# AE-HYU/monte_carlo_localization

Hardware: AMD Instinct MI355X
Metric: MCL updates/sec (particle*beam/s) (higher is better)
Workload: dtype f64; 1 GPU; 4194304 particles/GPU x 1081 beams, Spielberg_map (2000x2000 @ 0.05796), initial cloud N((0.0, 0.0, 0.0),(0.5 m,0.5 m,0.4 rad)) (tracking regime), action (0.05, 0.0, 0.01), stock sensor/motion params, multinomial resampling, Philox seed 42; the timed updates follow 5 warm-up updates (the particle set has resampled to motion-noise width); particles_total=4194304, beams=1081, parallelism=single GPU

## Files before the change

### monte_carlo_localization_amd/csrc/mcl_engine.hip

```cpp
#include "../../include/mcl_hip_engine.h"

#include <hip/hip_runtime.h>
#include <hip/hip_ext.h>
#include <rocprim/device/device_radix_sort.hpp>

#include <algorithm>
#include <chrono>
#include <cmath>
#include <cstdio>
#include <cstring>
#include <string>
#include <vector>

#include "mcl_engine_internal.h"
#include "mcl_kernels.h"
#include "mcl_host_math.h"
#include "mcl_lfield.h"

static_assert(MCL_WEDGES == mcl::kWedges || MCL_KWEDGES != 16, "include/mcl_hip_engine.h and csrc/mcl_wedge.h disagree");

using namespace mcl_host;

namespace {

thread_local std::string g_create_error;

int ensure_lt(mcl_engine *h)
{
    size_t need = (size_t)(h->P + 1) * h->bpad;
    if (need > h->lt_capacity) {
        dfree(h->d_Lt);
        HIPCHK(h, hipMalloc(&h->d_Lt, 2 * need * sizeof(float)));
        h->lt_capacity = need;
    }
    h->ltd_cols = (h->B + 2 * h->beam_margin + 64) & ~63;
    const size_t need_d = (size_t)mcl::sweep_table_rows(h->P) * h->ltd_cols;
    if (need_d > h->ltd_capacity) {
        dfree(h->d_Ltd);
        HIPCHK(h, hipMalloc(&h->d_Ltd, need_d * sizeof(double)));
        h->ltd_capacity = need_d;
        h->ltd_ready = false;
    }
    return MCL_OK;
}

void build_ltd(mcl_engine *h);

int weight_stats(mcl_engine *h, bool from_log, const double *d_max_override, bool defer_sums = false)
{
    const int64_t n = h->N;
    const double *src = from_log ? h->d_logw : h->d_w;
    const double *max_parts = nullptr;
    if (!d_max_override) {
        if (!(from_log && h->max_partials_ready))
            hipLaunchKernelGGL(mcl::k_reduce_max, dim3(mcl::kRedBlocks), dim3(mcl::kRedThreads), 0, h->stream, src, n, h->d_maxpart);
        max_parts = h->d_maxpart;
    }
    h->max_partials_ready = false;
    hipLaunchKernelGGL(mcl::k_weights, dim3(mcl::kRedBlocks), dim3(mcl::kRedThreads), 0, h->stream, src, from_log ? 1 : 0,
                       d_max_override ? d_max_override : h->d_scalars, h->d_x[h->cur], h->d_y[h->cur], h->d_th[h->cur], n, h->d_w, h->d_q, h->d_part,
                       (from_log && h->cfg.resample_neff_permille > 0) ? h->d_carry[h->carry_idx ^ 1] : (double *)nullptr,
                       max_parts, mcl::kRedBlocks);
    h->carry_pending = from_log && h->cfg.resample_neff_permille > 0;
    if (!from_log) h->carry_valid = false;
    if (defer_sums) h->sums_pending = true;
    else hipLaunchKernelGGL(mcl::k_final_sums, dim3(1), dim3(mcl::kRedThreads), 0, h->stream, h->d_part, mcl::kRedBlocks, h->d_scalars);
    HIPCHK(h, hipGetLastError());
    return MCL_OK;
}

int fetch_scalars(mcl_engine *h)
{
    HIPCHK(h, hipMemcpyAsync(h->h_result, h->d_result, kResultWords * 8, hipMemcpyDeviceToHost, h->stream));
    HIPCHK(h, hipStreamSynchronize(h->stream));
    unpack_result(h);
    return MCL_OK;
}

bool sweep_hybrid(const mcl_engine *h)
{
    return h->sweep_global && h->env_sweep_hybrid != 0 && h->rec_ok && h->sweep_hyb_layout_ok && h->d_beam_err != nullptr &&
           h->d_distw != nullptr && h->d_distg != nullptr && (size_t)mcl::kSwWinBytes + (size_t)h->ltd_cols * 8 <= 80 * 1024 - 64;
}

bool sweep_far_expected(const mcl_engine *h) { return h->far_fresh || h->h_result[15] >= mcl::kFarWindowedMin / 2; }
bool sweep_hybrid_decide(mcl_engine *h)
{
    if (!sweep_hybrid(h)) return false;
    if (h->env_sweep_hybrid == 2) return true;
    if (h->far_fresh) { h->hyb_backoff = 0; h->hyb_skip = 0; return false; }
    if (h->last_sweep_global == 2) {
        if (h->h_result[15] >= mcl::kFarWindowedMin / 2) { h->hyb_backoff = h->hyb_backoff ? std::min(32, 2 * h->hyb_backoff) : 1; h->hyb_skip = h->hyb_backoff; }
        else h->hyb_backoff = 0;
    }
    if (h->hyb_skip > 0) { --h->hyb_skip; return false; }
    return true;
}

int sweep_play(const mcl_engine *h, bool hybrid)
{
    if (hybrid) return mcl::kSwSide - (mcl::kSwHybReach + 2) - 3;
    if (h->sweep_global) return 1 << 20;
    return mcl::kSwSide - (h->P + 2) - 3;
}

int64_t max_sweep_units(int64_t n) { return (n + mcl::kSwUnit - 1) / mcl::kSwUnit + mcl::kSwMaxCuts + 2; }

int launch_sweep_plan(mcl_engine *h, int64_t n, int nwg, int g, bool hybrid)
{
    const int ngroups = mcl::kWedges / g;
    const size_t need = (size_t)max_sweep_units(n) * ngroups;
    if (need > h->items_capacity) {
        dfree(h->d_items); dfree(h->d_centres);
        h->items_capacity = 0;
        HIPCHK(h, hipMalloc(&h->d_items, need * sizeof(int4)));
// ... 284 lines not shown
            a.far_sorted = h->d_far_sorted;
            a.far_windowed = sweep_far_expected(h) ? 1 : 0;
            h->far_fresh = false;
            a.far_list = h->d_far_list; a.far_count = h->d_result + 15;
        }
        const bool sweep_hyb = sweep && sweep_hyb_now;
        const bool sweep_glob = sweep && h->sweep_global && !sweep_hyb;
        const bool sweep_rec = sweep && h->rec_ok && h->sweep_rec_layout_ok && h->d_beam_err != nullptr &&
                               (size_t)mcl::kSwWinBytes + (size_t)h->ltd_cols * 8 <= 80 * 1024 - 64;
        const bool sweep_pairs = sweep_rec && !sweep_hyb && (h->env_sweep_pairs >= 0 ? h->env_sweep_pairs != 0 : (sweep_glob || a.far_windowed != 0));
        size_t qlds = sweep ? (sweep_glob ? 0 : (size_t)mcl::kSwWinBytes) + (sweep_rec ? (size_t)h->ltd_cols * 8 : 0) : (size_t)h->qside * h->qside;
        h->last_sweep_global = sweep_glob ? 1 : (sweep_hyb ? 2 : 0); h->last_sweep_rec = sweep_rec ? 1 : 0; h->last_sweep_pairs = (sweep_rec && (sweep_glob || sweep_pairs)) ? 1 : 0;
        dim3 qg((unsigned)nseg);
        unsigned long long *d_dbg = nullptr;
        const char *dbgpath = h->env_debug_wg.empty() ? nullptr : h->env_debug_wg.c_str();
        if (dbgpath) { HIPCHK(h, hipMalloc(&d_dbg, (size_t)qg.x * 32)); HIPCHK(h, hipMemset(d_dbg, 0, (size_t)qg.x * 32)); a.dbg = d_dbg; }
        dim3 gfar((unsigned)std::max<int64_t>(1, std::min<int64_t>(4 * (int64_t)h->num_cu, (n + 15) / 16)));
        const int fix_split = std::max(1, std::min(16, (8 * h->num_cu) / std::max(nseg, 1)));
        if (!sweep) HIPCHK(h, hipEventRecord(h->ev[EV_K0], h->stream));
        if (count) {
            if (sweep_hyb) hipExtLaunchKernelGGL((mcl::k_rays_sweep<true, false, true, false, true>), qg, b, qlds, h->stream, nullptr, h->ev[EV_K1], 0, a);
            else if (sweep_glob && sweep_rec) hipExtLaunchKernelGGL((mcl::k_rays_sweep<true, true, true, true>), qg, b, qlds, h->stream, nullptr, h->ev[EV_K1], 0, a);
            else if (sweep_glob) hipExtLaunchKernelGGL((mcl::k_rays_sweep<true, true>), qg, b, qlds, h->stream, nullptr, h->ev[EV_K1], 0, a);
            else if (sweep && sweep_rec && sweep_pairs) hipExtLaunchKernelGGL((mcl::k_rays_sweep<true, false, true, true>), qg, b, qlds, h->stream, nullptr, h->ev[EV_K1], 0, a);
            else if (sweep && sweep_rec) hipExtLaunchKernelGGL((mcl::k_rays_sweep<true, false, true>), qg, b, qlds, h->stream, nullptr, h->ev[EV_K1], 0, a);
            else if (sweep) hipExtLaunchKernelGGL((mcl::k_rays_sweep<true>), qg, b, qlds, h->stream, nullptr, h->ev[EV_K1], 0, a);
#ifdef MCL_LEGACY_RAY_KERNELS
            else if (cell) hipLaunchKernelGGL((mcl::k_rays_cell<true>), qg, b, qlds, h->stream, a);
            else hipLaunchKernelGGL((mcl::k_rays_quad<true>), qg, b, qlds, h->stream, a);
#endif
            if (!sweep) HIPCHK(h, hipEventRecord(h->ev[EV_K1], h->stream));
            if (sweep && a.far_windowed) { const int rcw = launch_far_windowed(h, a, n, true); if (rcw) return rcw; }
            hipLaunchKernelGGL((mcl::k_rays_far<true>), gfar, b, 0, h->stream, a);
            hipLaunchKernelGGL((mcl::k_rays_fix<true>), dim3(nseg * fix_split), dim3(256), 0, h->stream, a);
            hipLaunchKernelGGL((mcl::k_rays_exact<true>), dim3(2 * h->num_cu), dim3(256), 0, h->stream, a);
        } else {
            if (sweep_hyb) hipExtLaunchKernelGGL((mcl::k_rays_sweep<false, false, true, false, true>), qg, b, qlds, h->stream, nullptr, h->ev[EV_K1], 0, a);
            else if (sweep_glob && sweep_rec) hipExtLaunchKernelGGL((mcl::k_rays_sweep<false, true, true, true>), qg, b, qlds, h->stream, nullptr, h->ev[EV_K1], 0, a);
            else if (sweep_glob) hipExtLaunchKernelGGL((mcl::k_rays_sweep<false, true>), qg, b, qlds, h->stream, nullptr, h->ev[EV_K1], 0, a);
            else if (sweep && sweep_rec && sweep_pairs) hipExtLaunchKernelGGL((mcl::k_rays_sweep<false, false, true, true>), qg, b, qlds, h->stream, nullptr, h->ev[EV_K1], 0, a);
            else if (sweep && sweep_rec) hipExtLaunchKernelGGL((mcl::k_rays_sweep<false, false, true>), qg, b, qlds, h->stream, nullptr, h->ev[EV_K1], 0, a);
            else if (sweep) hipExtLaunchKernelGGL((mcl::k_rays_sweep<false>), qg, b, qlds, h->stream, nullptr, h->ev[EV_K1], 0, a);
#ifdef MCL_LEGACY_RAY_KERNELS
            else if (cell) hipLaunchKernelGGL((mcl::k_rays_cell<false>), qg, b, qlds, h->stream, a);
            else hipLaunchKernelGGL((mcl::k_rays_quad<false>), qg, b, qlds, h->stream, a);
#endif
            if (!sweep) HIPCHK(h, hipEventRecord(h->ev[EV_K1], h->stream));
            if (sweep && a.far_windowed) { const int rcw = launch_far_windowed(h, a, n, false); if (rcw) return rcw; }
            hipLaunchKernelGGL((mcl::k_rays_far<false>), gfar, b, 0, h->stream, a);
            hipLaunchKernelGGL((mcl::k_rays_fix<false>), dim3(nseg * fix_split), dim3(256), 0, h->stream, a);
            hipLaunchKernelGGL((mcl::k_rays_exact<false>), dim3(2 * h->num_cu), dim3(256), 0, h->stream, a);
        }
        if (sweep) {
            hipExtLaunchKernelGGL(mcl::k_combine_logw, dim3(mcl::kRedBlocks), dim3(256), 0, h->stream, nullptr, h->ev[EV_RAYS], 0, n, h->d_perm, h->d_logw_acc,
                                  h->d_logw, h->d_maxpart, h->d_fix_count, nseg, segcap, h->d_fix_over);
            h->ev_rays_bound = true;
            h->max_partials_ready = true;
        } else {
            hipLaunchKernelGGL(mcl::k_fix_overflow, dim3(1), dim3(256), 0, h->stream, h->d_fix_count, nseg, segcap, h->d_fix_over);
            hipLaunchKernelGGL(mcl::k_gather_logw, dim3((unsigned)((n + 255) / 256)), dim3(256), 0, h->stream, h->d_logw_acc, n, h->d_logw);
        }
        if (d_dbg) {
            std::vector<unsigned long long> hd((size_t)qg.x * 4);
            HIPCHK(h, hipStreamSynchronize(h->stream));
            HIPCHK(h, hipMemcpy(hd.data(), d_dbg, hd.size() * 8, hipMemcpyDeviceToHost));
            if (FILE *f = fopen(dbgpath, "wb")) { fwrite(hd.data(), 8, hd.size(), f); fclose(f); }
            (void)hipFree(d_dbg);
        }
        h->last_quad = true;
    } else if (count) {
        hipLaunchKernelGGL((mcl::k_rays_skip<1, true>), g, b, lds, h->stream, a);
    } else {
        switch (R) {
        case 1: hipLaunchKernelGGL((mcl::k_rays_skip<1, false>), g, b, lds, h->stream, a); break;
        case 2: hipLaunchKernelGGL((mcl::k_rays_skip<2, false>), g, b, lds, h->stream, a); break;
        case 3: hipLaunchKernelGGL((mcl::k_rays_skip<3, false>), g, b, lds, h->stream, a); break;
        default: hipLaunchKernelGGL((mcl::k_rays_skip<4, false>), g, b, lds, h->stream, a); break;
        }
    }
    if (!windows && !h->capturing && !direct_table) HIPCHK(h, hipEventRecord(h->ev[EV_K1], h->stream));
    h->last_mode = mode;
    h->prep_folded = false;
    h->layout_stale_used = false; h->keys_done = false;
    if (!h->capturing) h->pc_ready = false;
    HIPCHK(h, hipGetLastError());
    return MCL_OK;
}

void stage_observation(mcl_engine *h, const float *obs, int stride)
{
    h->ltd_ready = false;
    for (int j = 0; j < h->B; ++j) h->h_obs[j] = obs[(size_t)j * stride];
}

void build_ltd(mcl_engine *h)
{
    dim3 gd((h->ltd_cols + 255) / 256, mcl::sweep_table_rows(h->P));
    hipLaunchKernelGGL(mcl::k_build_ltd, gd, dim3(256), 0, h->stream, h->d_L, h->d_obs_idx, h->B, h->ltd_cols, h->P, h->beam_margin, h->d_Ltd);
    h->ltd_ready = true;
}

int upload_observation(mcl_engine *h)
{
    HIPCHK(h, hipMemcpyAsync(h->d_obs, h->h_obs, (size_t)h->B * sizeof(float), hipMemcpyHostToDevice, h->stream));
    int rc = h->capturing ? MCL_OK : ensure_lt(h);
    if (rc) return rc;
    dim3 g((h->bpad + 255) / 256, h->P + 1);
    hipLaunchKernelGGL(mcl::k_obs_build_lt, g, dim3(256), 0, h->stream, h->d_obs, h->res, h->P, h->d_L, h->B, h->bpad, h->d_obs_idx, h->d_Lt,
// ... 143 lines not shown
    const int nb = mcl_host::lf_used_beams(h, obs, stride, h->h_lf_beams);
    if (nb > 0)
        HIPCHK(h, hipMemcpyAsync(h->d_lf_beams, h->h_lf_beams, (size_t)nb * sizeof(double2), hipMemcpyHostToDevice, h->stream));
    HIPCHK(h, hipEventRecord(h->ev[EV_QUERY], h->stream));
    HIPCHK(h, hipEventRecord(h->ev[EV_K0], h->stream));
    const int rc = mcl_host::launch_lfield_on(h, h->d_x[h->cur], h->d_y[h->cur], h->d_th[h->cur], n, h->d_lf_beams, nb, h->d_logw);
    if (rc != MCL_OK) return rc;
    HIPCHK(h, hipEventRecord(h->ev[EV_K1], h->stream));
    h->max_partials_ready = false;
    h->last_quad = false;
    h->last_lf = true;
    return MCL_OK;
}

}

int mcl_host::fail(mcl_engine *h, int code, const char *msg) { if (h) h->err = msg; return code; }
int mcl_host::fail(mcl_engine *h, int code, const std::string &msg) { return fail(h, code, msg.c_str()); }

std::string &mcl_host::create_error() { return g_create_error; }

bool mcl_host::ready(mcl_engine *h, bool need_particles)
{
    return h && h->have_map && h->B > 0 && (!need_particles || h->have_particles);
}

float mcl_host::elapsed(hipEvent_t a, hipEvent_t b)
{
    float ms = 0.f;
    (void)hipEventElapsedTime(&ms, a, b);
    return ms;
}

void mcl_host::graph_reset(mcl_engine *h)
{
    for (int k = 0; k < 2; ++k)
        if (h->graph_exec[k]) { (void)hipGraphExecDestroy(h->graph_exec[k]); h->graph_exec[k] = nullptr; }
    h->graph_warm = false;
    h->prep_cache_valid = false; h->prep_folded = false;
    h->layout_valid = false; h->layout_stale_used = false; h->keys_done = false;
    h->pc_ready = false;
}

int mcl_host::scan_weights(mcl_engine *h, const uint64_t *d_q, uint64_t *d_cdf, int64_t n, uint64_t offset, uint64_t *d_total)
{
    int nb = (int)((n + mcl::kScanTile - 1) / mcl::kScanTile);
    mcl::CompactOut co{};
    const bool own = d_q == h->d_q && d_cdf == h->d_cdf && offset == 0 && !h->env_no_compact && h->d_ccdf;
    if (own) {
        co.block_cnt = h->d_blockcnt; co.ccdf = h->d_ccdf; co.cidx = h->d_cidx; co.crec = h->d_crec; co.ctop = h->d_ctop;
        co.x = h->d_x[h->cur]; co.y = h->d_y[h->cur]; co.th = h->d_th[h->cur];
        co.cap = (uint32_t)h->compact_cap; co.total = h->d_result + 16;
    }
    hipLaunchKernelGGL(mcl::k_scan_partials, dim3(nb), dim3(mcl::kScanThreads), 0, h->stream, d_q, n, h->d_blocktot, co.block_cnt);
    const bool fold = h->sums_pending && d_q == h->d_q;
    hipLaunchKernelGGL(mcl::k_scan_spine, dim3(1), dim3(1024), 0, h->stream, h->d_blocktot, nb, offset, d_total, co.block_cnt, co.total,
                       fold ? h->d_part : (const double *)nullptr, mcl::kRedBlocks, h->d_scalars);
    if (fold) h->sums_pending = false;
    const size_t nlead = (size_t)((n + 15) >> mcl::kLeaderShift) + 1;
    if (nlead > h->leaders_capacity) {
        graph_reset(h);
        dfree(h->d_leaders);
        HIPCHK(h, hipMalloc(&h->d_leaders, nlead * 8));
        h->leaders_capacity = nlead;
    }
    if (h->bind_sensor_event && own && !h->capturing) {
        hipExtLaunchKernelGGL(mcl::k_scan_final, dim3(nb), dim3(mcl::kScanThreads), 0, h->stream, nullptr, h->ev[EV_SENSOR], 0, d_q, n, h->d_blocktot, d_cdf,
                              h->d_leaders, co);
        h->ev_sensor_bound = true; h->bind_sensor_event = false;
    } else {
        hipLaunchKernelGGL(mcl::k_scan_final, dim3(nb), dim3(mcl::kScanThreads), 0, h->stream, d_q, n, h->d_blocktot, d_cdf, h->d_leaders, co);
    }
    HIPCHK(h, hipGetLastError());
    h->blocktot_for = d_cdf; h->blocktot_n = n;
    if (d_cdf == h->d_cdf) { h->compact_n = -1; h->compact_pending = own; h->list_epoch++; }
    return MCL_OK;
}

void mcl_host::unpack_result(mcl_engine *h)
{
    std::memcpy(h->h_scalars, h->h_result, 8 * sizeof(double));
    std::memcpy(h->h_counters, h->h_result + 8, 4 * sizeof(unsigned long long));
    h->h_fix_count = h->h_result[12];
    uint64_t qt;
    std::memcpy(&qt, &h->h_scalars[2], 8);
    h->q_total = qt;
    h->global_sums[0] = h->h_scalars[1];
    h->global_sums[1] = h->h_scalars[3];
    h->global_sums[2] = h->h_scalars[4];
    h->global_sums[3] = h->h_scalars[5];
    h->global_sums[4] = h->h_scalars[6];
    if (h->compact_pending) {
        const unsigned long long na = h->h_result[16];
        h->compact_n = na <= (unsigned long long)h->compact_cap ? (int64_t)na : -1;
        h->compact_pending = false;
    }
}

int mcl_abi_version(void) { return MCL_ABI_VERSION; }

const char *mcl_last_error(const mcl_engine_t *h) { return h ? h->err.c_str() : g_create_error.c_str(); }

int mcl_create(const mcl_config_t *cfg, mcl_engine_t **out)
{
    if (cfg && (cfg->resample_neff_permille < 0 || cfg->resample_neff_permille > 1000)) return MCL_ERR_INVALID_ARG;
    g_create_error.clear();
    if (!cfg || !out) { g_create_error = "null argument"; return MCL_ERR_INVALID_ARG; }
// ... 2022 lines not shown
```

### monte_carlo_localization_amd/csrc/mcl_engine_internal.h

```cpp
#pragma once
#include "../../include/mcl_hip_engine.h"

#include <hip/hip_runtime.h>
#include <hip/hip_ext.h>

#include <cstdint>
#include <string>
#include <vector>

#include "mcl_types.h"
#include "mcl_host_math.h"

enum { EV_START = 0, EV_RESAMPLE, EV_QUERY, EV_RAYS, EV_SENSOR, EV_K0, EV_K1, EV_COUNT };


constexpr unsigned long long kExactCap = 1ull << 16;
constexpr int kResultWords = 18;
constexpr int kResultStage = 40;
constexpr int kResultStamp = 32;
constexpr int kCompactEntryBytes = 44;

struct mcl_comm;
void comm_free(struct mcl_comm *c);
void comm_forget(struct mcl_comm *c);
// ... 71 lines not shown
    mcl::PrepClear prep_cache{};
    bool prep_cache_valid = false, prep_folded = false;
    int64_t prep_cache_n = 0;
    bool max_partials_ready = false;
    int4 *d_items = nullptr;
    int4 *d_centres = nullptr;
    size_t items_capacity = 0;
    int *d_nitems = nullptr;
    int64_t plan_n = 0;
    double4 *d_unit_sums = nullptr;
    uint32_t *d_unit_begin = nullptr;
    int *d_nunits = nullptr;
    size_t unit_sums_capacity = 0;
    int64_t env_cell_min = 0, env_cell_slice = 0;
    int env_qslices_per_cu = 0, env_qside = 0, env_sweep_g = 0;
    std::string env_debug_wg;

    int64_t cap = 0, N = 0;
    bool have_particles = false;
    double *d_x[2]{}, *d_y[2]{}, *d_th[2]{};
    int cur = 0;
    double *d_w = nullptr, *d_logw = nullptr, *d_tmp = nullptr;
    double *d_carry[2]{};
    int carry_idx = 0;
    bool carry_valid = false, carry_pending = false;
    bool resampled_last = true;
    hipGraphExec_t graph_exec[2] = {nullptr, nullptr};
    bool graph_warm = false;
    bool capturing = false;
    double *d_logw_acc = nullptr;
    uint64_t *d_q = nullptr, *d_cdf = nullptr, *d_blocktot = nullptr;
    uint32_t *d_bm = nullptr;
    uint64_t *d_bm_pop = nullptr, *d_bm_pref = nullptr;
    size_t bm_capacity = 0;
    uint32_t *d_blockcnt = nullptr;
    uint64_t *d_ccdf = nullptr, *d_ctop = nullptr;
    uint32_t *d_cidx = nullptr;
    double4 *d_crec = nullptr;
    int64_t compact_cap = 0;
    int64_t compact_n = -1;
    bool compact_pending = false;
    bool compact_used = false;
    uint64_t *d_gcdf = nullptr, *d_gtop = nullptr;
    size_t gcdf_capacity = 0;
    int env_no_compact = 0;
    uint64_t *d_leaders = nullptr;
    size_t leaders_capacity = 0;
    double4 *d_pack[2]{};
    bool pack_valid[2] = {false, false};
    int32_t *d_idx = nullptr;
    uint8_t *d_steps = nullptr;
    size_t steps_capacity = 0, blocktot_capacity = 0;
    const uint64_t *blocktot_for = nullptr;
    int64_t blocktot_n = 0;
    double *d_part = nullptr;
    double *d_maxpart = nullptr;
    bool sums_pending = false;
    double *d_scalars = nullptr;
    unsigned long long *d_counters = nullptr;
    double *d_inject = nullptr;
    double4 *d_pc = nullptr;
    short4 *d_qr = nullptr;
    bool quad_ok = false;
    int qside = 0;
    unsigned long long *d_fix_list = nullptr, *d_fix_count = nullptr, *d_fix_over = nullptr;
    unsigned long long *d_exact_list = nullptr;
    unsigned long long fix_cap = 0, fix_alloc = 0;
    size_t fix_count_alloc = 0;
    int fix_segments = 0;
    uint8_t *d_far = nullptr;
    uint32_t *d_far_list = nullptr;
    uint32_t *d_far_sorted = nullptr, *d_far_cnt = nullptr;
    double4 *d_pcs = nullptr;
    double *d_ths = nullptr;
    uint8_t *d_distw = nullptr;
    uint32_t *d_perm = nullptr, *d_skey = nullptr, *d_srank = nullptr;
    uint32_t *d_skey2 = nullptr, *d_sval2 = nullptr;
    void *d_sort_tmp = nullptr;
    size_t sort_tmp_bytes = 0;
    int env_sort_radix = -1;
    uint32_t *d_tile_used = nullptr;
    uint32_t *d_hist = nullptr, *d_histpart = nullptr;
    int *d_bbox = nullptr;
    uint32_t *d_cut_start = nullptr, *d_cut_end = nullptr;
    bool env_no_bucket_cuts = false;
    int *d_tilemap = nullptr, *d_tilemark = nullptr;
    int *d_bbox_nx = nullptr, *d_tilemap_nx = nullptr, *d_tilemark_nx = nullptr;
    hipEvent_t ev_children = nullptr, ev_layout = nullptr;
    hipEvent_t ev_ext_in = nullptr, ev_ext_out = nullptr;
    bool stage_async_rays = false, stage_async_weights = false;
    bool stage_kept = false;
    struct mcl_comm *comm = nullptr;
    unsigned long long list_epoch = 0;
    bool layout_valid = false, layout_pending = false;
    int64_t layout_n = 0;
    bool ev_resample_bound = false, ev_rays_bound = false, ev_sensor_bound = false, ev_query_skipped = false;
    bool bind_sensor_event = false;
    bool layout_wanted = false;
    bool layout_stale_used = false;
    bool keys_done = false;
    bool env_no_stale_layout = false;
    bool env_comm_no_lists = false;
    bool env_comm_no_pregather = false;
    mcl::PrepClear prep_passed{};
    double2 *d_slice_mean = nullptr;
    size_t slice_mean_capacity = 0;
// ... 119 lines not shown
```

### monte_carlo_localization_amd/csrc/mcl_kernels.h

```cpp
#pragma once
#include "mcl_types.h"
#include <type_traits>
#include "mcl_ray_core.h"
#include "mcl_device_math.h"
#include "mcl_wedge.h"
#include "mcl_motion.h"

namespace mcl {

constexpr int kRedBlocks = 1024;
constexpr int kRedThreads = 256;
__device__ __forceinline__ void final_sums_of(const double *__restrict__ part, int nb, double *__restrict__ scalars, double (*sm)[7]);


__device__ __forceinline__ uint64_t wave_incl_scan_u64(uint64_t v, int lane)
{
#pragma unroll
    for (int o = 1; o < 64; o <<= 1) {
        uint64_t t = (uint64_t)__shfl_up((long long)v, o, 64);
        if (lane >= o) v += t;
    }
    return v;
}

// ... 1699 lines not shown
            const int s0 = d0 > 1 ? d0 : 1;
            int ja, jb, ja2;
            quad_ranges(qr, q, a.B, ja, jb, ja2);
            for (int seg = 0; seg < 2; ++seg)
            for (int j0 = seg ? ja2 : ja, je = seg ? a.B : jb; j0 < je; j0 += 64) {
                int j = j0 + lane;
                if (j < je) {
                    int r = a.P;
                    unsigned np = 0;
                    uint32_t amb = amb0;
                    if (sane) {
                        double2 cs = a.beam_cs[j];
                        double ux = cth * cs.x - sth * cs.y;
                        double uy = sth * cs.x + cth * cs.y;
                        r = trace_fp64<false, COUNT>(a, nullptr, 0, base, p0x, p0y, ux, uy, s0, amb, np, field);
                    }
                    if (!sane || amb < kGuard || a.force_exact == 1) {
                        r = march_exact(a, a.x[i], a.y[i], a.th[i] + (double)a.beam_angle[j]);
                        ++cnt_exact;
                    }
                    acc += (double)a.Lt[(size_t)r * a.bpad + j];
                    if (a.steps || a.steps16) store_step(a, i, j, r);
                    if (COUNT) cnt_probe += np;
                }
            }
        }
        acc = wave_sum(acc);
        if (lane == 0) atomicAdd(&a.logw[p], acc);
      }
    }
    if (a.counters) {
        cnt_exact = wave_sum_u64(cnt_exact);
        cnt_off = wave_sum_u64(cnt_off);
        cnt_probe = wave_sum_u64(cnt_probe);
        if (lane == 0) {
            if (cnt_exact) atomicAdd(&a.counters[0], cnt_exact);
            if (cnt_off) atomicAdd(&a.counters[1], cnt_off);
            if (COUNT && cnt_probe) atomicAdd(&a.counters[2], cnt_probe);
        }
    }
}

__global__ void k_product_weights(const uint8_t *__restrict__ steps, const uint16_t *__restrict__ steps16, const int32_t *__restrict__ obs_idx, int64_t n, int B,
                                  const double *__restrict__ table , int tw, double inv_squash,
                                  double *__restrict__ w_out)
{
    int64_t i = (int64_t)blockIdx.x * blockDim.x + threadIdx.x;
    if (i >= n) return;
    double w = 1.0;
    for (int j = 0; j < B; ++j) w *= table[(size_t)(steps16 ? (int)steps16[(size_t)i * B + j] : (int)steps[(size_t)i * B + j]) * tw + obs_idx[j]];
    w_out[i] = pow(w, inv_squash);
}

__global__ __launch_bounds__(kRedThreads) void k_reduce_max(const double *__restrict__ v, int64_t n, double *__restrict__ part)
{
    __shared__ double sm[kRedThreads / 64];
    double m = -INFINITY;
    for (int64_t i = (int64_t)blockIdx.x * kRedThreads + threadIdx.x; i < n; i += (int64_t)gridDim.x * kRedThreads)
        m = fmax(m, v[i]);
    m = wave_max(m);
    if ((threadIdx.x & 63) == 0) sm[threadIdx.x >> 6] = m;
    __syncthreads();
    if (threadIdx.x == 0) {
        for (int k = 1; k < kRedThreads / 64; ++k) m = fmax(m, sm[k]);
        part[blockIdx.x] = m;
    }
}
__global__ __launch_bounds__(kRedThreads) void k_final_max(const double *__restrict__ part, int nb, double *__restrict__ out,
                                                           double *__restrict__ out2)
{
    __shared__ double sm[kRedThreads / 64];
    double m = -INFINITY;
    for (int i = threadIdx.x; i < nb; i += kRedThreads) m = fmax(m, part[i]);
    m = wave_max(m);
    if ((threadIdx.x & 63) == 0) sm[threadIdx.x >> 6] = m;
    __syncthreads();
    if (threadIdx.x == 0) {
        for (int k = 1; k < kRedThreads / 64; ++k) m = fmax(m, sm[k]);
        out[0] = m;
        if (out2) out2[0] = m;
    }
}

__global__ void k_copy_double(const double *__restrict__ src, double *__restrict__ dst) { dst[0] = src[0]; }
__global__ void k_set_double(double *__restrict__ dst, double v) { dst[0] = v; }
__global__ void k_spin_ms(double ms)
{
    const unsigned long long t0 = __builtin_amdgcn_s_memrealtime();
    const unsigned long long ticks = (unsigned long long)((ms < 2000.0 ? ms : 2000.0) * 1e5);
    while (__builtin_amdgcn_s_memrealtime() - t0 < ticks) __builtin_amdgcn_s_sleep(64);
}

__global__ void k_group_max(GroupMaxArgs a)
{
    double m = -INFINITY;
    for (int i = 0; i < a.n; ++i) m = fmax(m, a.src[i][0]);
    a.out[0] = m;
}

__global__ void k_stage_pack(const unsigned long long *__restrict__ res, double *__restrict__ vec, int n_shards, int self, int listed,
                             unsigned long long list_cap)
{
    const int len = 5 + 3 * n_shards + 2;
    const double *sc = reinterpret_cast<const double *>(res);
    for (int i = threadIdx.x; i < len; i += blockDim.x) {
        double v = 0.0;
        if (i == 0) v = sc[1];
        else if (i < 5) v = sc[2 + i];
        else if (i == 5 + 3 * self) v = (listed && res[16] <= list_cap) ? (double)(res[16] + 1ull) : 0.0;
        else if (i == 6 + 3 * self) v = (double)(res[2] & 0xFFFFFFFFull);
        else if (i == 7 + 3 * self) v = (double)(res[2] >> 32);
        else if (i == len - 2) v = res[12] != 0ull ? 1.0 : 0.0;
        else if (i == len - 1) v = sc[7];
        vec[i] = v;
    }
}

__global__ __launch_bounds__(kRedThreads) void k_weights(const double *__restrict__ logw_or_w, int from_log,
                                                        const double *__restrict__ maxp, const double *__restrict__ x,
                                                        const double *__restrict__ y, const double *__restrict__ th, int64_t n,
                                                        double *__restrict__ w_out, uint64_t *__restrict__ q_out,
                                                        double *__restrict__ part ,
                                                        double *__restrict__ carry_out ,
                                                        const double *__restrict__ max_parts = nullptr, int n_max_parts = 0)
{
    __shared__ double sm[kRedThreads / 64][7];
    double mx;
    if (max_parts) {
        __shared__ double mxs[kRedThreads / 64];
        double m = -INFINITY;
        for (int i = threadIdx.x; i < n_max_parts; i += kRedThreads) m = fmax(m, max_parts[i]);
        m = wave_max(m);
        if ((threadIdx.x & 63) == 0) mxs[threadIdx.x >> 6] = m;
        __syncthreads();
        mx = mxs[0];
        for (int k = 1; k < kRedThreads / 64; ++k) mx = fmax(mx, mxs[k]);
        if (blockIdx.x == 0 && threadIdx.x == 0) const_cast<double *>(maxp)[0] = mx;
    } else {
        mx = *maxp;
    }
    double sw = 0, swx = 0, swy = 0, sws = 0, swc = 0, sww = 0;
    uint64_t sq = 0;
    for (int64_t i = (int64_t)blockIdx.x * kRedThreads + threadIdx.x; i < n; i += (int64_t)gridDim.x * kRedThreads) {
        double w, wq;
        if (from_log) {
            const double lw = logw_or_w[i];
            const double d = lw == -INFINITY ? -INFINITY : lw - mx;
            w = det_exp(d); wq = w; if (carry_out) carry_out[i] = d;
        }
        else {
            w = logw_or_w[i];
            wq = (mx > 0.0 && w > 0.0) ? (w / mx) : 0.0;
        }
        uint64_t q = (uint64_t)(wq * kWeightScale);
        w_out[i] = w;
        q_out[i] = q;
        double s, c;
        sincos(th[i], &s, &c);
        sw += w; sq += q; swx += w * x[i]; swy += w * y[i]; sws += w * s; swc += w * c; sww += w * w;
    }
    sw = wave_sum(sw); swx = wave_sum(swx); swy = wave_sum(swy); sws = wave_sum(sws); swc = wave_sum(swc); sww = wave_sum(sww);
    sq = wave_sum_u64(sq);
    int wv = threadIdx.x >> 6;
    if ((threadIdx.x & 63) == 0) {
        sm[wv][0] = sw; sm[wv][1] = __longlong_as_double((long long)sq); sm[wv][2] = swx; sm[wv][3] = swy; sm[wv][4] = sws; sm[wv][5] = swc; sm[wv][6] = sww;
    }
    __syncthreads();
    if (threadIdx.x == 0) {
        uint64_t tq = 0;
        double t[7] = {0, 0, 0, 0, 0, 0, 0};
        for (int k = 0; k < kRedThreads / 64; ++k) {
            t[0] += sm[k][0]; tq += (uint64_t)__double_as_longlong(sm[k][1]);
            t[2] += sm[k][2]; t[3] += sm[k][3]; t[4] += sm[k][4]; t[5] += sm[k][5]; t[6] += sm[k][6];
        }
        double *p = part + (size_t)blockIdx.x * 8;
        p[0] = t[0]; p[1] = __longlong_as_double((long long)tq); p[2] = t[2]; p[3] = t[3]; p[4] = t[4]; p[5] = t[5]; p[6] = t[6];
    }
}
__device__ __forceinline__ void final_sums_of(const double *__restrict__ part, int nb, double *__restrict__ scalars, double (*sm)[7])
{
    const bool mine = threadIdx.x < kRedThreads;
    double t[7] = {0, 0, 0, 0, 0, 0, 0};
    uint64_t tq = 0;
    if (mine)
        for (int i = threadIdx.x; i < nb; i += kRedThreads) {
            const double *p = part + (size_t)i * 8;
            t[0] += p[0]; tq += (uint64_t)__double_as_longlong(p[1]); t[2] += p[2]; t[3] += p[3]; t[4] += p[4]; t[5] += p[5]; t[6] += p[6];
        }
    t[0] = wave_sum(t[0]); t[2] = wave_sum(t[2]); t[3] = wave_sum(t[3]); t[4] = wave_sum(t[4]); t[5] = wave_sum(t[5]); t[6] = wave_sum(t[6]);
    tq = wave_sum_u64(tq);
    int wv = threadIdx.x >> 6;
    if (mine && (threadIdx.x & 63) == 0) {
        sm[wv][0] = t[0]; sm[wv][1] = __longlong_as_double((long long)tq); sm[wv][2] = t[2]; sm[wv][3] = t[3]; sm[wv][4] = t[4]; sm[wv][5] = t[5]; sm[wv][6] = t[6];
    }
    __syncthreads();
    if (threadIdx.x == 0) {
        double r[7] = {0, 0, 0, 0, 0, 0, 0};
        uint64_t rq = 0;
        for (int k = 0; k < kRedThreads / 64; ++k) {
            r[0] += sm[k][0]; rq += (uint64_t)__double_as_longlong(sm[k][1]);
            r[2] += sm[k][2]; r[3] += sm[k][3]; r[4] += sm[k][4]; r[5] += sm[k][5]; r[6] += sm[k][6];
        }
        scalars[1] = r[0]; scalars[2] = __longlong_as_double((long long)rq);
        scalars[3] = r[2]; scalars[4] = r[3]; scalars[5] = r[4]; scalars[6] = r[5];
        scalars[7] = r[6];
    }
}
__global__ __launch_bounds__(kRedThreads) void k_final_sums(const double *__restrict__ part, int nb, double *__restrict__ scalars)
{
    __shared__ double sm[kRedThreads / 64][7];
    final_sums_of(part, nb, scalars, sm);
}
// ... 139 lines not shown
```

### monte_carlo_localization_amd/csrc/mcl_rays_sweep.h

```cpp
#pragma once

namespace mcl {

constexpr int kSwUnder = 127;
constexpr int kSwUnit = 1024;
constexpr int kSwFx = 32;
constexpr int kSwSide = 256;
#ifndef MCL_SW_PITCH
#define MCL_SW_PITCH 260
#endif
constexpr int kSwPitch = MCL_SW_PITCH;
static_assert(kSwPitch >= kSwSide && (kSwPitch % 4) == 0, "window rows are written as dwords");
constexpr int kSwWinBytes = kSwSide * kSwPitch;
#ifndef MCL_SW_HYB_PLAY
#define MCL_SW_HYB_PLAY 40
#endif
constexpr int kSwHybPlay = MCL_SW_HYB_PLAY;
constexpr int kSwHybReach = kSwSide - (kSwHybPlay + 3) - 2;
#if MCL_KWEDGES == 8
__device__ constexpr double kSwHybInvDx[2] = {1.0, 1.414213562373095};
__device__ constexpr double kSwHybInvDy[2] = {1.4142135623730951, 1.0};
#elif MCL_KWEDGES == 16
__device__ constexpr double kSwHybInvDx[4] = {1.0, 1.082392200292394, 1.414213562373095, 2.6131259297527527};
__device__ constexpr double kSwHybInvDy[4] = {2.613125929752753, 1.4142135623730951, 1.082392200292394, 1.0};
// ... 913 lines not shown
                        const bool over = __builtin_usub_overflow((uint32_t)rem, by, &nr);
                        go = !over;
                        rem = (int)nr;
                        cnt_probe += (go && valid) ? 1 : 0;
                    } while (go && ++trips <= ((GLOBAL || HYB) ? (int)cdinit : 300));
                    if (go) g = 0u;
                }
                if (COUNT && valid) ++cnt_probe;
                const uint32_t thr = expired ? 0xFFFFFFFFu : gthresh;
                const bool amb = valid && g < thr;
                lt_pending = 0.0;
                if (valid && !amb) {
                    const int left = rem > 0 ? rem : 0;
                    lt_pending = *reinterpret_cast<const double *>(reinterpret_cast<const char *>(a.Ltd) +
                                                                   mad_u24_s((uint32_t)(left + kSwUnder), st8, (uint32_t)(jcur + a.beam_margin) << 3));
                    if (want_steps) store_step(a, (int64_t)i, jcur, a.P - left);
                }
                if (amb) {
                    const unsigned int fslot = atomicAdd(&fixn_sh, 1u);
                    if (fslot < a.fix_cap) fix_seg[fslot] = ((unsigned long long)sl << 16) | (unsigned long long)jcur;
                }
            }
            acc += lt_pending;
        }
        if (live && walk_n > 0 && (expired_fast || gwalk < gthresh)) {
            const int jr0 = n1 > 0 ? ja : ja2, jr1 = n1 > 0 ? jb : a.B;
            for (int k = 0; k < walk_n; ++k) {
                const int jamb = jwalk + walk_t0 + k;
                if (jamb < jr0 || jamb >= jr1) continue;
                const unsigned int fslot = atomicAdd(&fixn_sh, 1u);
                if (fslot < a.fix_cap) fix_seg[fslot] = ((unsigned long long)sl << 16) | (unsigned long long)(jamb & 0xFFFF);
            }
            acc_fast = 0.0;
        }
        if (have) atomicAdd(&a.logw[slot], acc_fast + acc);
    }
    }
    }
    __syncthreads();
    if (a.dbg && threadIdx.x == 0) {
        unsigned long long *d = a.dbg + (size_t)blockIdx.x * 4;
        d[0] = dbg_t0; d[1] = __builtin_amdgcn_s_memrealtime(); d[2] = dbg_items | (dbg_bar << 32); d[3] = dbg_wait;
    }
    if (threadIdx.x == 0) a.fix_count[(size_t)blockIdx.x * 8] = fixn_sh;
    if (COUNT && a.counters) {
        cnt_probe = wave_sum_u64(cnt_probe);
        if (lane == 0 && cnt_probe) atomicAdd(&a.counters[2], cnt_probe);
    }
}

__global__ __launch_bounds__(256) void k_combine_logw(int64_t n, const uint32_t *__restrict__ perm, const double *__restrict__ acc,
                                                     double *__restrict__ logw, double *__restrict__ maxpart,
                                                     const unsigned long long *__restrict__ fix_counts, int nseg, unsigned long long fix_cap,
                                                     unsigned long long *__restrict__ over)
{
    __shared__ double sm[4];
    __shared__ unsigned int over_sh;
    if (blockIdx.x == 0 && over) {
        if (threadIdx.x == 0) over_sh = 0u;
        __syncthreads();
        unsigned int c = 0;
        for (int k = threadIdx.x; k < nseg; k += blockDim.x) c += fix_counts[(size_t)k * 8] > fix_cap ? 1u : 0u;
        if (c) atomicAdd(&over_sh, c);
        __syncthreads();
        if (threadIdx.x == 0) *over = over_sh;
    }
    double m = -INFINITY;
    const int64_t stride = (int64_t)gridDim.x * blockDim.x;
    int64_t s = (int64_t)blockIdx.x * blockDim.x + threadIdx.x;
    for (; s + 3 * stride < n; s += 4 * stride) {
        const double v0 = acc[s], v1 = acc[s + stride], v2 = acc[s + 2 * stride], v3 = acc[s + 3 * stride];
        const uint32_t i0 = perm[s], i1 = perm[s + stride], i2 = perm[s + 2 * stride], i3 = perm[s + 3 * stride];
        logw[i0] = v0; logw[i1] = v1; logw[i2] = v2; logw[i3] = v3;
        m = fmax(fmax(m, v0), fmax(fmax(v1, v2), v3));
    }
    for (; s < n; s += stride) {
        const double v = acc[s];
        logw[perm[s]] = v;
        m = fmax(m, v);
    }
    m = wave_max(m);
    if ((threadIdx.x & 63) == 0) sm[threadIdx.x >> 6] = m;
    __syncthreads();
    if (threadIdx.x == 0) maxpart[blockIdx.x] = fmax(fmax(sm[0], sm[1]), fmax(sm[2], sm[3]));
}

}
```

Baseline: 862.4 billion particle*beam/s.

## Fold scan tile totals into weights kernel, skipping the scan-partials pass

The weights kernel now accumulates per-scan-tile sums of quantized weights and nonzero counts with wave reductions and atomics. This lets the resampling scan skip its separate k_scan_partials pass over d_q. The tile accumulators are zeroed inside the preceding combine or reduce-max kernel, and host-side state tracks when the totals are valid. The cost is atomics on every wave plus added bookkeeping, and the risk of stale totals if the state flags get out of sync.

```diff
diff --git a/monte_carlo_localization_amd/csrc/mcl_engine.hip b/monte_carlo_localization_amd/csrc/mcl_engine.hip
--- a/monte_carlo_localization_amd/csrc/mcl_engine.hip
+++ b/monte_carlo_localization_amd/csrc/mcl_engine.hip
@@ -51,16 +51,26 @@
     const int64_t n = h->N;
     const double *src = from_log ? h->d_logw : h->d_w;
     const double *max_parts = nullptr;
+    const int ntiles = (int)((n + mcl::kScanTile - 1) / mcl::kScanTile);
+    bool tiles = false;
     if (!d_max_override) {
-        if (!(from_log && h->max_partials_ready))
-            hipLaunchKernelGGL(mcl::k_reduce_max, dim3(mcl::kRedBlocks), dim3(mcl::kRedThreads), 0, h->stream, src, n, h->d_maxpart);
+        if (!(from_log && h->max_partials_ready)) {
+            tiles = defer_sums && n <= h->cap;
+            hipLaunchKernelGGL(mcl::k_reduce_max, dim3(mcl::kRedBlocks), dim3(mcl::kRedThreads), 0, h->stream, src, n, h->d_maxpart,
+                               tiles ? h->d_blocktot : (uint64_t *)nullptr, h->d_blockcnt, ntiles);
+        } else {
+            tiles = defer_sums && h->tiles_zeroed_n == n && h->tiles_zeroed_ptr == h->d_blocktot;
+        }
         max_parts = h->d_maxpart;
     }
     h->max_partials_ready = false;
     hipLaunchKernelGGL(mcl::k_weights, dim3(mcl::kRedBlocks), dim3(mcl::kRedThreads), 0, h->stream, src, from_log ? 1 : 0,
                        d_max_override ? d_max_override : h->d_scalars, h->d_x[h->cur], h->d_y[h->cur], h->d_th[h->cur], n, h->d_w, h->d_q, h->d_part,
                        (from_log && h->cfg.resample_neff_permille > 0) ? h->d_carry[h->carry_idx ^ 1] : (double *)nullptr,
-                       max_parts, mcl::kRedBlocks);
+                       max_parts, mcl::kRedBlocks, tiles ? h->d_blocktot : (uint64_t *)nullptr, h->d_blockcnt);
+    h->tiles_zeroed_n = -1;
+    h->tiles_ready_n = tiles ? n : -1;
+    if (tiles) h->blocktot_for = nullptr;
     h->carry_pending = from_log && h->cfg.resample_neff_permille > 0;
     if (!from_log) h->carry_valid = false;
     if (defer_sums) h->sums_pending = true;
@@ -451,8 +461,13 @@
             hipLaunchKernelGGL((mcl::k_rays_exact<false>), dim3(2 * h->num_cu), dim3(256), 0, h->stream, a);
         }
         if (sweep) {
+            const bool zero_tiles = n <= h->cap;
             hipExtLaunchKernelGGL(mcl::k_combine_logw, dim3(mcl::kRedBlocks), dim3(256), 0, h->stream, nullptr, h->ev[EV_RAYS], 0, n, h->d_perm, h->d_logw_acc,
-                                  h->d_logw, h->d_maxpart, h->d_fix_count, nseg, segcap, h->d_fix_over);
+                                  h->d_logw, h->d_maxpart, h->d_fix_count, nseg, segcap, h->d_fix_over,
+                                  zero_tiles ? h->d_blocktot : (uint64_t *)nullptr, h->d_blockcnt, (int)((n + mcl::kScanTile - 1) / mcl::kScanTile));
+            h->tiles_zeroed_n = zero_tiles ? n : -1; h->tiles_zeroed_ptr = h->d_blocktot;
+            h->tiles_ready_n = -1;
+            if (zero_tiles) h->blocktot_for = nullptr;
             h->ev_rays_bound = true;
             h->max_partials_ready = true;
         } else {
@@ -702,7 +717,10 @@
         co.x = h->d_x[h->cur]; co.y = h->d_y[h->cur]; co.th = h->d_th[h->cur];
         co.cap = (uint32_t)h->compact_cap; co.total = h->d_result + 16;
     }
-    hipLaunchKernelGGL(mcl::k_scan_partials, dim3(nb), dim3(mcl::kScanThreads), 0, h->stream, d_q, n, h->d_blocktot, co.block_cnt);
+    const bool have_totals = d_q == h->d_q && h->tiles_ready_n == n;
+    h->tiles_ready_n = -1; h->tiles_zeroed_n = -1;
+    if (!have_totals)
+        hipLaunchKernelGGL(mcl::k_scan_partials, dim3(nb), dim3(mcl::kScanThreads), 0, h->stream, d_q, n, h->d_blocktot, co.block_cnt);
     const bool fold = h->sums_pending && d_q == h->d_q;
     hipLaunchKernelGGL(mcl::k_scan_spine, dim3(1), dim3(1024), 0, h->stream, h->d_blocktot, nb, offset, d_total, co.block_cnt, co.total,
                        fold ? h->d_part : (const double *)nullptr, mcl::kRedBlocks, h->d_scalars);
diff --git a/monte_carlo_localization_amd/csrc/mcl_engine_internal.h b/monte_carlo_localization_amd/csrc/mcl_engine_internal.h
--- a/monte_carlo_localization_amd/csrc/mcl_engine_internal.h
+++ b/monte_carlo_localization_amd/csrc/mcl_engine_internal.h
@@ -147,6 +147,8 @@
     uint8_t *d_steps = nullptr;
     size_t steps_capacity = 0, blocktot_capacity = 0;
     const uint64_t *blocktot_for = nullptr;
+    int64_t tiles_zeroed_n = -1, tiles_ready_n = -1;
+    const uint64_t *tiles_zeroed_ptr = nullptr;
     int64_t blocktot_n = 0;
     double *d_part = nullptr;
     double *d_maxpart = nullptr;
diff --git a/monte_carlo_localization_amd/csrc/mcl_kernels.h b/monte_carlo_localization_amd/csrc/mcl_kernels.h
--- a/monte_carlo_localization_amd/csrc/mcl_kernels.h
+++ b/monte_carlo_localization_amd/csrc/mcl_kernels.h
@@ -1775,9 +1775,16 @@
     w_out[i] = pow(w, inv_squash);
 }
 
-__global__ __launch_bounds__(kRedThreads) void k_reduce_max(const double *__restrict__ v, int64_t n, double *__restrict__ part)
+__device__ __forceinline__ void tile_totals_clear(uint64_t *__restrict__ zero_tot, uint32_t *__restrict__ zero_cnt, int nz)
+{
+    if (!zero_tot) return;
+    for (int64_t k = (int64_t)blockIdx.x * blockDim.x + threadIdx.x; k < nz; k += (int64_t)gridDim.x * blockDim.x) { zero_tot[k] = 0ull; zero_cnt[k] = 0u; }
+}
+__global__ __launch_bounds__(kRedThreads) void k_reduce_max(const double *__restrict__ v, int64_t n, double *__restrict__ part,
+                                                           uint64_t *__restrict__ zero_tot = nullptr, uint32_t *__restrict__ zero_cnt = nullptr, int nz = 0)
 {
     __shared__ double sm[kRedThreads / 64];
+    tile_totals_clear(zero_tot, zero_cnt, nz);
     double m = -INFINITY;
     for (int64_t i = (int64_t)blockIdx.x * kRedThreads + threadIdx.x; i < n; i += (int64_t)gridDim.x * kRedThreads)
         m = fmax(m, v[i]);
@@ -1845,7 +1852,8 @@
                                                         double *__restrict__ w_out, uint64_t *__restrict__ q_out,
                                                         double *__restrict__ part ,
                                                         double *__restrict__ carry_out ,
-                                                        const double *__restrict__ max_parts = nullptr, int n_max_parts = 0)
+                                                        const double *__restrict__ max_parts = nullptr, int n_max_parts = 0,
+                                                        uint64_t *__restrict__ tile_tot = nullptr, uint32_t *__restrict__ tile_cnt = nullptr)
 {
     __shared__ double sm[kRedThreads / 64][7];
     double mx;
@@ -1864,7 +1872,12 @@
     }
     double sw = 0, swx = 0, swy = 0, sws = 0, swc = 0, sww = 0;
     uint64_t sq = 0;
-    for (int64_t i = (int64_t)blockIdx.x * kRedThreads + threadIdx.x; i < n; i += (int64_t)gridDim.x * kRedThreads) {
+    static_assert(kScanTile % 64 == 0 && kRedThreads % 64 == 0, "a wave's 64 particles lie in one scan tile");
+    const int lane = threadIdx.x & 63;
+    for (int64_t i0 = (int64_t)blockIdx.x * kRedThreads + (threadIdx.x - lane); i0 < n; i0 += (int64_t)gridDim.x * kRedThreads) {
+        const int64_t i = i0 + lane;
+        uint64_t q = 0;
+        if (i < n) {
         double w, wq;
         if (from_log) {
             const double lw = logw_or_w[i];
@@ -1875,12 +1888,23 @@
             w = logw_or_w[i];
             wq = (mx > 0.0 && w > 0.0) ? (w / mx) : 0.0;
         }
-        uint64_t q = (uint64_t)(wq * kWeightScale);
+        q = (uint64_t)(wq * kWeightScale);
         w_out[i] = w;
         q_out[i] = q;
         double s, c;
         sincos(th[i], &s, &c);
         sw += w; sq += q; swx += w * x[i]; swy += w * y[i]; sws += w * s; swc += w * c; sww += w * w;
+        }
+        if (tile_tot) {
+            const unsigned long long alive = __ballot(q != 0ull);
+            if (alive) {
+                const uint64_t t = wave_sum_u64(q);
+                if (lane == 0) {
+                    atomicAdd(reinterpret_cast<unsigned long long *>(tile_tot) + i0 / kScanTile, (unsigned long long)t);
+                    atomicAdd(tile_cnt + i0 / kScanTile, (uint32_t)__popcll(alive));
+                }
+            }
+        }
     }
     sw = wave_sum(sw); swx = wave_sum(swx); swy = wave_sum(swy); sws = wave_sum(sws); swc = wave_sum(swc); sww = wave_sum(sww);
     sq = wave_sum_u64(sq);
diff --git a/monte_carlo_localization_amd/csrc/mcl_rays_sweep.h b/monte_carlo_localization_amd/csrc/mcl_rays_sweep.h
--- a/monte_carlo_localization_amd/csrc/mcl_rays_sweep.h
+++ b/monte_carlo_localization_amd/csrc/mcl_rays_sweep.h
@@ -989,10 +989,12 @@
 __global__ __launch_bounds__(256) void k_combine_logw(int64_t n, const uint32_t *__restrict__ perm, const double *__restrict__ acc,
                                                      double *__restrict__ logw, double *__restrict__ maxpart,
                                                      const unsigned long long *__restrict__ fix_counts, int nseg, unsigned long long fix_cap,
-                                                     unsigned long long *__restrict__ over)
+                                                     unsigned long long *__restrict__ over,
+                                                     uint64_t *__restrict__ zero_tot = nullptr, uint32_t *__restrict__ zero_cnt = nullptr, int nz = 0)
 {
     __shared__ double sm[4];
     __shared__ unsigned int over_sh;
+    tile_totals_clear(zero_tot, zero_cnt, nz);
     if (blockIdx.x == 0 && over) {
         if (threadIdx.x == 0) over_sh = 0u;
         __syncthreads();
```

Result: no change. 861.0 billion particle*beam/s (-0.2%).
